# tari-project/bulletproofs-plus

Measured on AMD Instinct MI355X. Metric: 64-bit range proofs verified/sec (batch), higher is better.
Workload: dtype u32

## Files before the change

### bulletproofs-plus_amd/_build.py

```python
import os
import subprocess
import sys

HERE = os.path.dirname(os.path.abspath(__file__))
CSRC = os.path.join(HERE, "csrc")
LIB = os.path.join(HERE, "libbpp_hip.so")
HOSTTEST_LIB = os.path.join(HERE, "libbpp_hosttest.so")
SOURCES = ["engine.hip"]
HEADERS = sorted(f for f in os.listdir(CSRC) if f.endswith((".h", ".inc"))) + [os.path.join("..", "..", "include", "bpp.h")]


def _stale(target, deps):
    if not os.path.exists(target):
        return True
    t = os.path.getmtime(target)
    return any(os.path.getmtime(d) > t for d in deps if os.path.exists(d))


def hipcc_path():
    for cand in (os.environ.get("HIPCC"), "/opt/rocm/bin/hipcc", "hipcc"):
        if cand and (os.path.isabs(cand) and os.path.exists(cand) or not os.path.isabs(cand)):
            return cand
    return "hipcc"

# ... 189 lines not shown
def build_refill_mixed_harness(force=False):
    src = os.path.join(CSRC, "hosttest_refill_mixed.cpp")
    deps = [src] + [os.path.join(CSRC, h) for h in HEADERS]
    if not force and not _stale(REFILL_MIXED_SANITIZER_BIN, deps):
        return REFILL_MIXED_SANITIZER_BIN
    subprocess.run(["g++", "-O1", "-g", "-std=c++17", "-fsanitize=address,undefined", "-fno-sanitize-recover=undefined",
                    "-fno-omit-frame-pointer", "-o", REFILL_MIXED_SANITIZER_BIN, src], check=True, cwd=CSRC)
    return REFILL_MIXED_SANITIZER_BIN


ITEM_STATES_SANITIZER_BIN = os.path.join(HERE, "hosttest_item_states_asan")


def build_item_states_harness(force=False):
    src = os.path.join(CSRC, "hosttest_item_states.cpp")
    deps = [src] + [os.path.join(CSRC, h) for h in HEADERS]
    if not force and not _stale(ITEM_STATES_SANITIZER_BIN, deps):
        return ITEM_STATES_SANITIZER_BIN
    subprocess.run(["g++", "-O1", "-g", "-std=c++17", "-fsanitize=address,undefined", "-fno-sanitize-recover=undefined",
                    "-fno-omit-frame-pointer", "-o", ITEM_STATES_SANITIZER_BIN, src], check=True, cwd=CSRC)
    return ITEM_STATES_SANITIZER_BIN


if __name__ == "__main__":
    build(force="--force" in sys.argv, verbose=True)
    build_hosttest(force="--force" in sys.argv)
```

### bulletproofs-plus_amd/csrc/engine.hip

```cpp
#include <hip/hip_runtime.h>
#include <stdio.h>
#include <string.h>
#include <time.h>

#include <algorithm>
#include <array>
#include <atomic>
#include <chrono>
#include <condition_variable>
#include <deque>
#include <functional>
#include <map>
#include <set>
#include <memory>
#include <mutex>
#include <string>
#include <thread>
#include <vector>

#include "../../include/bpp.h"
#include "chain_dev.h"
#include "chain_host.h"
#include "ct.h"
#include "kernels_prove.h"
#include "kernels_verify.h"
#include "lanes_host.h"
#include "msm.h"
#include "msm_plain.h"
#include "prove_job_host.h"
#include "prove_pack_host.h"
#include "runtime_host.h"
#include "upload_host.h"
#include "ingest.h"
#include "ingest_mixed.h"
#include "verdict.h"
#include "refill.h"
#include "refill_mixed.h"
#include "item_states.h"

using namespace bpp;

namespace {

struct EngineError {
  int code;
  std::string msg;
};

#define HIP_CHECK(expr)                                                                          \
// ... 339 lines not shown
#define BPP_REFILLED_MSG "the batch was refilled on the stream (bpp_batch_refill_enqueue) and takes enqueued calls only: upload the arrays for a blocking call"

void adopt_buffers(Batch &dst, Batch &src) {
#define BPP_ADOPT(f) dst.f.swap(src.f)
  BPP_ADOPT(d_ext_status); BPP_ADOPT(bytes); BPP_ADOPT(states); BPP_ADOPT(seeds); BPP_ADOPT(d_desc); BPP_ADOPT(minvals);
  BPP_ADOPT(src_off); BPP_ADOPT(owner); BPP_ADOPT(idx_commit); BPP_ADOPT(idx_proof); BPP_ADOPT(status0); BPP_ADOPT(chal);
  BPP_ADOPT(rows); BPP_ADOPT(parts); BPP_ADOPT(gemm_lo); BPP_ADOPT(gemm_hi); BPP_ADOPT(gparts); BPP_ADOPT(gemm_mult); BPP_ADOPT(scal); BPP_ADOPT(shr); BPP_ADOPT(tab); BPP_ADOPT(rng_out); BPP_ADOPT(weights); BPP_ADOPT(chain_wide);
  BPP_ADOPT(masks); BPP_ADOPT(chal_bytes); BPP_ADOPT(status); BPP_ADOPT(group_first); BPP_ADOPT(group_dlo); BPP_ADOPT(dynpts); BPP_ADOPT(dyn_hi); BPP_ADOPT(dec_spill);
  BPP_ADOPT(msm.counts); BPP_ADOPT(msm.starts); BPP_ADOPT(msm.sorted); BPP_ADOPT(msm.order); BPP_ADOPT(msm.order_win);
  BPP_ADOPT(msm.cls_hist);
  BPP_ADOPT(msm.buckets); BPP_ADOPT(msm.Q); BPP_ADOPT(msm.W); BPP_ADOPT(msm.R); BPP_ADOPT(msm.comp32);
  BPP_ADOPT(msm.is_identity); BPP_ADOPT(msm.term_sidx); BPP_ADOPT(msm.term_pidx); BPP_ADOPT(msm.group_off);
  BPP_ADOPT(h_rng); BPP_ADOPT(h_weights); BPP_ADOPT(h_wide); BPP_ADOPT(h_status); BPP_ADOPT(h_status_any); BPP_ADOPT(h_ident); BPP_ADOPT(h_masks); BPP_ADOPT(h_states);
#undef BPP_ADOPT
  dst.h_status_dirty.swap(src.h_status_dirty);
  std::swap(dst.h_status_dirty_of, src.h_status_dirty_of);
  if (!src.status_settled) std::fill(dst.h_status_dirty.begin(), dst.h_status_dirty.end(), (uint8_t)1);
}

void wipe_batch_secrets(Batch &b, hipStream_t s);

}

struct PipeJob {
  uint64_t ticket = 0;
  int action = 0;
  size_t chunk = 0;
  std::shared_ptr<Params> Pp;
  uint64_t params = 0;
  UploadPlan pl;
  size_t n_items = 0;
  uint32_t t = 0;
  int rc = 0;
  std::string err;
  std::vector<uint8_t> masks, present;
  bool done = false;
};

struct PipeLane {
  bpp_ctx *child = nullptr;
  std::thread th;
  std::shared_ptr<PipeJob> job;
  bool busy = false;
};

struct Pipeline {
  std::mutex mu;
  std::condition_variable cv;
  std::mutex submit_mu;
  std::vector<std::unique_ptr<PipeLane>> lanes;
  std::map<uint64_t, std::shared_ptr<PipeJob>> tickets;
  uint64_t next_ticket = 1;
  uint32_t next_lane = 0;
  bool quit = false;
};

void pipeline_shutdown(bpp_ctx *ctx);

struct ProveJob;
using ProvePipeline = lanes::TicketLanes<bpp_ctx *, ProveJob>;
void prove_pipeline_shutdown(bpp_ctx *ctx);
int prove_pipeline_check_stats(bpp_ctx *ctx, struct bpp_prove_check_stats *sum);
int prove_pipeline_recovery_stats(bpp_ctx *ctx, uint64_t *replayed, uint64_t *mismatched);
int prove_pipeline_secret_bytes(bpp_ctx *ctx, uint64_t *examined, uint64_t *nonzero);

enum MsmReduce : uint32_t { MSM_RC_QUAD = 0, MSM_RC2 = 1, MSM_RC = 2, MSM_BITSUM = 3 };
struct MsmForm {
  bool valid = false;
  bool plain = false;
  bool ct = false;
  bool quad = false;
  MsmReduce reduce = MSM_RC_QUAD;
  bool final_quad = false;
  bool narrow = false;
  uint32_t dig_cap = 0;
  uint32_t slices = 0;
  uint32_t c = 0, K = 0, K_wide = 0, nb = 0, G = 0, terms = 0;
};

struct CtMsmWork {
// ... 42 lines not shown
  bool ev_wait_ready = false;
  WaitHint wait_hint_rng, wait_hint_end, wait_hint_prove;
  hipStream_t side_stream = nullptr;
  hipEvent_t ev_fork, ev_join;
  hipStream_t chain_stream = nullptr;
  hipEvent_t ev_chain_fork, ev_chain_done;
  DevBuf<Strobe> d_chain_t0;
  PinnedBuf<uint32_t> h_chain_zero;
  uint64_t device_chain_calls = 0, device_chain_redraws = 0, wide_chain_calls = 0;
  DevBuf<uint8_t> scratch128;
  DevBuf<uint8_t> prove_arena;
  PinnedBuf<uint8_t> prove_pin_in, prove_pin_out;
  std::vector<hipStream_t> prove_streams;
  std::vector<hipStream_t> prove_lane_streams;
  hipStream_t prove_msm_stream = nullptr;
  std::vector<hipEvent_t> prove_sync_events;
  std::vector<hipStream_t> prove_aux_streams;
  std::vector<hipEvent_t> prove_aux_events;
  std::vector<hipEvent_t> prove_events;
  bpp_prove_profile pprof{};
  struct Options {
    int transcripts_wave = -1, tables_wave = -1, side_decompress = -1, msm_c_bias = -1, msm_c_max = -1, msm_c_add = -1, msm_rc2 = -1, msm_quad = -1, msm_final_quad = -1,
        fb_threads = -1, prove_subs = -1, msm_split = -1, fused_columns = -1, prove_prio = -1, prove_fused = -1, static_gemm = -1, lazy_columns = -1, ct = -1, prove_parts = -1, prove_waves = -1, prove_fifo = -1, chain = -1, chain_test_zero = 0, wait = -1, ct_back = -1, chain_inline = -1, wide_in_lanes = -1,
        prove_check = -1, prove_check_recovery = -1, msm_plain = -1, verify_check = -1, msm_ct_k = -1, verify_joint = 0, msm_prelude_slices = 0;
  } opt;
  struct bpp_verify_check_stats vcheck_stats{};
  int verify_check_off = 0;
  struct bpp_verify_joint_stats vjoint_stats{};
  WaitHint wait_hint_fallback;
  struct VerifyTamper {
    int passes = 0, group = 0, kind = 0;
  } vtamper;
  std::unique_ptr<Batch> check_spare;
  WaitHint check_hint_rng, check_hint_end;
  struct bpp_prove_check_stats check_stats{};
  PinnedBuf<uint8_t> check_pin;
  DevBuf<uint8_t> check_dev;
  PinnedBuf<uint32_t> check_words;
  uint64_t check_replayed = 0, check_mismatched = 0;
  const void *check_zeroed_seeds = nullptr, *check_zeroed_masks = nullptr;
  size_t check_zeroed_seeds_n = 0, check_zeroed_masks_n = 0;
  std::mutex check_note_mu;
  std::vector<std::array<uint8_t, 32>> check_recovery_failed;
  struct CheckTamper {
    int proof = 0, byte = 1, mask = 1, times = 1, nonce = 0;
  } tamper;
  std::vector<hipEvent_t> enq_events;
// ... 38 lines not shown
    {"msm_split", "BPP_MSM_SPLIT", &bpp_ctx::Options::msm_split},
    {"fused_columns", "BPP_FUSED_COLUMNS", &bpp_ctx::Options::fused_columns},
    {"prove_prio", "BPP_PROVE_PRIO", &bpp_ctx::Options::prove_prio},
    {"prove_fused", "BPP_PROVE_FUSED", &bpp_ctx::Options::prove_fused},
    {"ct", "BPP_CT", &bpp_ctx::Options::ct},
    {"ct_back", "BPP_CT_BACK", &bpp_ctx::Options::ct_back},
    {"prove_parts", "BPP_PROVE_PARTS", &bpp_ctx::Options::prove_parts},
    {"prove_waves", "BPP_PROVE_WAVES", &bpp_ctx::Options::prove_waves},
    {"prove_fifo", "BPP_PROVE_FIFO", &bpp_ctx::Options::prove_fifo},
    {"static_gemm", "BPP_STATIC_GEMM", &bpp_ctx::Options::static_gemm},
    {"lazy_columns", "BPP_LAZY_COLUMNS", &bpp_ctx::Options::lazy_columns},
    {"chain", "BPP_CHAIN", &bpp_ctx::Options::chain},
    {"chain_test_zero", "BPP_CHAIN_TEST_ZERO", &bpp_ctx::Options::chain_test_zero},
    {"wait", "BPP_WAIT", &bpp_ctx::Options::wait},
    {"chain_inline", "BPP_CHAIN_INLINE", &bpp_ctx::Options::chain_inline},
    {"wide_in_lanes", "BPP_WIDE_IN_LANES", &bpp_ctx::Options::wide_in_lanes},
    {"prove_check", "BPP_PROVE_CHECK", &bpp_ctx::Options::prove_check},
    {"prove_check_recovery", "BPP_PROVE_CHECK_RECOVERY", &bpp_ctx::Options::prove_check_recovery},
    {"msm_plain", "BPP_MSM_PLAIN", &bpp_ctx::Options::msm_plain},
    {"verify_check", "BPP_VERIFY_CHECK", &bpp_ctx::Options::verify_check},
    {"msm_ct_k", "BPP_MSM_CT_K", &bpp_ctx::Options::msm_ct_k},
    {"verify_joint", "BPP_VERIFY_JOINT", &bpp_ctx::Options::verify_joint},
    {"msm_prelude_slices", "BPP_MSM_PRELUDE_SLICES", &bpp_ctx::Options::msm_prelude_slices},
};
struct TamperName {
  const char *name;
  int bpp_ctx::CheckTamper::*field;
};
const TamperName kTamperKnobs[] = {
    {"prove_check_tamper", &bpp_ctx::CheckTamper::proof},
    {"prove_check_tamper_byte", &bpp_ctx::CheckTamper::byte},
    {"prove_check_tamper_xor", &bpp_ctx::CheckTamper::mask},
    {"prove_check_tamper_times", &bpp_ctx::CheckTamper::times},
    {"prove_check_tamper_nonce", &bpp_ctx::CheckTamper::nonce},
};
struct VerifyTamperName {
  const char *name;
  int bpp_ctx::VerifyTamper::*field;
};
const VerifyTamperName kVerifyTamperKnobs[] = {
    {"verify_check_tamper", &bpp_ctx::VerifyTamper::passes},
    {"verify_check_tamper_group", &bpp_ctx::VerifyTamper::group},
    {"verify_check_tamper_kind", &bpp_ctx::VerifyTamper::kind},
};
void options_from_env(bpp_ctx *c) {
  for (const OptionName &o : kOptions)
// ... 981 lines not shown
  std::vector<uint32_t> first(n_groups + 1);
  for (size_t g = 0; g <= n_groups; g++) first[g] = (uint32_t)(g * n_per_group);
  run_weight_chains_generic(rng32_all, weights32_out, first.data(), (uint32_t)n_groups);
  return BPP_OK;
}

int bpp_weights_from_chain(const uint8_t *rng32_all, size_t n_total, uint8_t *weights32_out) {
  if ((!rng32_all || !weights32_out) && n_total) return BPP_ERR_INVALID_ARGUMENT;
  weights_from_chain_host(rng32_all, n_total, weights32_out);
  return BPP_OK;
}

}

namespace {

void wipe_batch_secrets(Batch &b, hipStream_t s) {
  if (b.seeds.p && b.seeds_dirty) (void)hipMemsetAsync(b.seeds.p, 0, b.seeds.n, s);
  if (b.masks.p && b.masks_dirty) (void)hipMemsetAsync(b.masks.p, 0, b.masks.n, s);
  b.seeds_dirty = b.masks_dirty = false;
}

void upload_host_pack(bpp_ctx *ctx, const Params &P, const bpp_verify_item *items, size_t n_items, const bpp_packed_batch *packed,
                      UploadPlan &pl) {
  const ParallelFor pf = [](uint32_t n, const std::function<void(uint32_t)> &fn) { host_parallel_for(n, fn); };
  const ParamShape shape{P.n_bits, P.m_max, P.t};
  std::vector<bpp_verify_item> synth;
  const bool arithmetic = packed && upload_pass_a_packed(*packed, pl, pf);
  if (packed && !arithmetic) {
    upload_packed_as_items(*packed, synth);
    items = synth.data();
    n_items = synth.size();
  }
  if (!arithmetic) upload_pass_a(items, n_items, pl);
  ctx->pin_upload.resize(pl.bytes_total + BPP_BYTES_SLACK);
  uint8_t *bytes = ctx->pin_upload.data();
  memset(bytes + pl.bytes_total, 0, BPP_BYTES_SLACK);
  if (arithmetic) upload_pass_b_packed(*packed, shape, pl, bytes, pf);
  else upload_pass_b(items, shape, pl, bytes, pf);
}

std::unique_ptr<Batch> new_batch(bpp_ctx *ctx) {
  auto B = std::make_unique<Batch>();
  if (ctx->spare_batch) {
    adopt_buffers(*B, *ctx->spare_batch);
    ctx->spare_batch.reset();
  }
  return B;
}

uint64_t upload_device(bpp_ctx *ctx, const std::shared_ptr<Params> &Pp, uint64_t params, UploadPlan &pl,
                       const uint8_t *const *challenges32, const uint8_t *rng_out32, std::unique_ptr<Batch> filled = nullptr) {
    Params &P = *Pp;
    const size_t n_items = pl.n_items;
    const bool resident = filled != nullptr;
    std::unique_ptr<Batch> B = resident ? std::move(filled) : new_batch(ctx);
    hipStream_t s = ctx->stream;
    SmallStaging L;
    bool registered = false;
// ... 2013 lines not shown
  *out = ctx->enq_stats;
  return BPP_OK;
}

int bpp_verify_batch_with_challenges(bpp_ctx *ctx, uint64_t params, const bpp_verify_item *items, size_t n_items,
                                     const uint8_t *const *challenges32, const uint8_t *rng_out32, int action, size_t chunk,
                                     uint8_t *masks_out, uint8_t *mask_present, char *errbuf, size_t errbuf_len) {
  auto upload = [&](uint64_t *h) -> int {
    BPP_ENTRY(ctx);
    if (!challenges32 || !rng_out32) return fail(ctx, BPP_ERR_INVALID_ARGUMENT, "null argument", errbuf, errbuf_len);
    return upload_impl(ctx, params, items, n_items, nullptr, h, challenges32, rng_out32, errbuf, errbuf_len);
  };
  return verify_uploaded(ctx, n_items, upload, action, chunk, masks_out, mask_present, errbuf, errbuf_len);
}

int bpp_verify_batch(bpp_ctx *ctx, uint64_t params, const bpp_verify_item *items, size_t n_items, int action,
                     size_t chunk, uint8_t *masks_out, uint8_t *mask_present, char *errbuf, size_t errbuf_len) {
  auto upload = [&](uint64_t *h) -> int { return bpp_batch_upload(ctx, params, items, n_items, h, errbuf, errbuf_len); };
  return verify_uploaded(ctx, n_items, upload, action, chunk, masks_out, mask_present, errbuf, errbuf_len);
}

int bpp_verify_batch_packed(bpp_ctx *ctx, uint64_t params, const bpp_packed_batch *in, int action, size_t chunk,
                            uint8_t *masks_out, uint8_t *mask_present, char *errbuf, size_t errbuf_len) {
  auto upload = [&](uint64_t *h) -> int { return bpp_batch_upload_packed(ctx, params, in, h, errbuf, errbuf_len); };
  return verify_uploaded(ctx, in ? in->n_items : SIZE_MAX, upload, action, chunk, masks_out, mask_present, errbuf, errbuf_len);
}

int bpp_verify_batch_packed_device(bpp_ctx *ctx, uint64_t params, const bpp_packed_batch *in, int action, size_t chunk,
                                   uint8_t *masks_out, uint8_t *mask_present, char *errbuf, size_t errbuf_len) {
  auto upload = [&](uint64_t *h) -> int { return bpp_batch_upload_packed_device(ctx, params, in, h, errbuf, errbuf_len); };
  return verify_uploaded(ctx, in ? in->n_items : SIZE_MAX, upload, action, chunk, masks_out, mask_present, errbuf, errbuf_len);
}

int bpp_verify_batch_mixed(bpp_ctx *ctx, uint64_t params, const bpp_mixed_batch *in, int action, size_t chunk, uint8_t *masks_out,
                           uint8_t *mask_present, char *errbuf, size_t errbuf_len) {
  auto upload = [&](uint64_t *h) -> int { return bpp_batch_upload_mixed(ctx, params, in, h, errbuf, errbuf_len); };
  return verify_uploaded(ctx, in ? in->n_items : SIZE_MAX, upload, action, chunk, masks_out, mask_present, errbuf, errbuf_len);
}

int bpp_verify_batch_mixed_device(bpp_ctx *ctx, uint64_t params, const bpp_mixed_batch *in, int action, size_t chunk,
                                  uint8_t *masks_out, uint8_t *mask_present, char *errbuf, size_t errbuf_len) {
  auto upload = [&](uint64_t *h) -> int { return bpp_batch_upload_mixed_device(ctx, params, in, h, errbuf, errbuf_len); };
  return verify_uploaded(ctx, in ? in->n_items : SIZE_MAX, upload, action, chunk, masks_out, mask_present, errbuf, errbuf_len);
}

int bpp_verify_batch_states(bpp_ctx *ctx, uint64_t params, const bpp_verify_item *items, size_t n_items, int action, size_t chunk,
// ... 85 lines not shown
  std::lock_guard<std::mutex> lk(init_mu);
  return slot;
}

template <class P, class F>
void pipeline_end(std::mutex &init_mu, std::shared_ptr<P> &slot, F on_uncollected) {
  std::shared_ptr<P> pp;
  {
    std::lock_guard<std::mutex> lk(init_mu);
    pp = std::move(slot);
    slot.reset();
  }
  if (!pp) return;
  pp->shutdown(on_uncollected);
  pp->for_each_lane([](bpp_ctx *c) { bpp_ctx_destroy(c); });
}

void pipe_worker(bpp_ctx *owner, Pipeline *pp, PipeLane *lane) {
  (void)hipSetDevice(owner->device);
  for (;;) {
    std::shared_ptr<PipeJob> job;
    {
      std::unique_lock<std::mutex> lk(pp->mu);
      pp->cv.wait(lk, [&] { return pp->quit || lane->job; });
      if (!lane->job) return;
      job = std::move(lane->job);
      lane->job.reset();
    }
    bpp_ctx *c = lane->child;
    char err[256];
    err[0] = 0;
    uint64_t h = 0;
    int rc = BPP_OK;
    GateHold gate(device_state(owner->device), job->n_items <= BPP_GATE_SMALL_PROOFS);
    {
      std::lock_guard<std::mutex> lk(c->mu);
      try {
        h = upload_device(c, job->Pp, job->params, job->pl, nullptr, nullptr);
      } catch (const EngineError &e) {
        rc = fail(c, e.code, e.msg, err, sizeof(err));
      } catch (const ProofErr &e) {
        rc = fail(c, e.code, e.msg, err, sizeof(err));
      } catch (const std::exception &e) {
        rc = fail(c, BPP_ERR_ENGINE, e.what(), err, sizeof(err));
      }
    }
    if (rc == BPP_OK) {
      const bool want_masks = job->action != BPP_VERIFY_ONLY;
      if (want_masks) {
        job->masks.assign(job->n_items * job->t * 32, 0);
        job->present.assign(job->n_items, 0);
      }
      rc = bpp_verify_resident(c, h, job->action, job->chunk, want_masks ? job->masks.data() : nullptr,
                               want_masks ? job->present.data() : nullptr, err, sizeof(err));
      (void)bpp_batch_destroy(c, h);
    }
    {
      std::lock_guard<std::mutex> lk(pp->mu);
      job->rc = rc;
      job->err = err;
      job->done = true;
      lane->busy = false;
    }
    pp->cv.notify_all();
  }
}

std::shared_ptr<Pipeline> make_pipeline(bpp_ctx *owner, const std::vector<bpp_ctx *> &children) {
  auto pp = std::make_shared<Pipeline>();
  for (bpp_ctx *c : children) {
    pp->lanes.push_back(std::make_unique<PipeLane>());
    pp->lanes.back()->child = c;
  }
  try {
    for (auto &lane : pp->lanes) lane->th = std::thread(pipe_worker, owner, pp.get(), lane.get());
  } catch (...) {
    {
      std::lock_guard<std::mutex> lk(pp->mu);
      pp->quit = true;
    }
    pp->cv.notify_all();
    for (auto &lane : pp->lanes)
      if (lane->th.joinable()) lane->th.join();
    throw;
  }
// ... 4 lines not shown

void pipeline_shutdown(bpp_ctx *ctx) {
  std::shared_ptr<Pipeline> pp;
  {
    std::lock_guard<std::mutex> lk(ctx->pipe_init_mu);
    pp = std::move(ctx->pipe);
    ctx->pipe.reset();
  }
  if (!pp) return;
  {
    std::unique_lock<std::mutex> lk(pp->mu);
    pp->cv.wait(lk, [&] {
      for (auto &l : pp->lanes)
        if (l->busy) return false;
      return true;
    });
    pp->quit = true;
  }
  pp->cv.notify_all();
  for (auto &l : pp->lanes) {
    if (l->th.joinable()) l->th.join();
    bpp_ctx_destroy(l->child);
  }
  std::lock_guard<std::mutex> lk(pp->mu);
  for (auto &kv : pp->tickets) wipe(kv.second->masks.data(), kv.second->masks.size());
  pp->tickets.clear();
}

extern "C" {

int bpp_ctx_pipeline_depth(bpp_ctx *ctx, uint32_t depth) {
  if (!ctx) return BPP_ERR_BAD_HANDLE;
  std::lock_guard<std::mutex> lk(ctx->pipe_init_mu);
  if (ctx->pipe) return fail(ctx, BPP_ERR_INVALID_ARGUMENT, "the pipeline is already running");
  if (depth < 1 || depth > 16) return fail(ctx, BPP_ERR_INVALID_ARGUMENT, "pipeline depth must be 1..16");
  ctx->pipe_depth = depth;
  return BPP_OK;
}

int bpp_verify_submit_packed(bpp_ctx *ctx, uint64_t params, const bpp_packed_batch *in, int action, size_t chunk,
                             uint64_t *ticket, char *errbuf, size_t errbuf_len) {
  if (!ctx) return BPP_ERR_BAD_HANDLE;
  if (hipSetDevice(ctx->device) != hipSuccess) return BPP_ERR_NO_DEVICE;
  try {
    if (!in || !ticket || in->n_items == 0)
      return fail(nullptr, BPP_ERR_INVALID_ARGUMENT, "Range statements or proofs length empty", errbuf, errbuf_len);
    if (action < 0 || action > 2) return fail(nullptr, BPP_ERR_INVALID_ARGUMENT, "unknown verify action", errbuf, errbuf_len);
    if (in->n_items > (1u << 24)) return fail(nullptr, BPP_ERR_SIZE_OVERFLOW, "batch too large", errbuf, errbuf_len);
    const std::shared_ptr<Params> Pp = params_registry().get(params);
    if (!Pp || Pp->device != ctx->device) return fail(nullptr, BPP_ERR_BAD_HANDLE, "unknown params handle", errbuf, errbuf_len);
    const std::shared_ptr<Pipeline> pp = pipeline_get(ctx, ctx->pipe_init_mu, ctx->pipe, ctx->pipe_depth, "pipeline lane: context creation failed",
                                                      [&](const std::vector<bpp_ctx *> &children) { return make_pipeline(ctx, children); });
    std::lock_guard<std::mutex> submit_lock(pp->submit_mu);
    PipeLane *lane;
    {
      std::unique_lock<std::mutex> lk(pp->mu);
      lane = pp->lanes[pp->next_lane].get();
      pp->cv.wait(lk, [&] { return !lane->busy; });
      lane->busy = true;
      pp->next_lane = (pp->next_lane + 1) % (uint32_t)pp->lanes.size();
    }
    auto job = std::make_shared<PipeJob>();
    job->action = action;
    job->chunk = chunk;
    job->Pp = Pp;
    job->params = params;
    job->n_items = in->n_items;
    job->t = Pp->t;
    try {
      upload_host_pack(lane->child, *Pp, nullptr, 0, in, job->pl);
    } catch (...) {
      secure_wipe(job->pl.seeds.data(), job->pl.seeds.size());
      {
        std::lock_guard<std::mutex> lk(pp->mu);
        lane->busy = false;
      }
      pp->cv.notify_all();
      throw;
    }
    {
      std::lock_guard<std::mutex> lk(pp->mu);
      job->ticket = pp->next_ticket++;
      pp->tickets[job->ticket] = job;
      lane->job = job;
      *ticket = job->ticket;
    }
    pp->cv.notify_all();
    return BPP_OK;
  }
  BPP_CATCH(nullptr, errbuf, errbuf_len)
}

int bpp_verify_collect(bpp_ctx *ctx, uint64_t ticket, uint8_t *masks_out, uint8_t *mask_present, char *errbuf,
                       size_t errbuf_len) {
  if (!ctx) return BPP_ERR_BAD_HANDLE;
  const std::shared_ptr<Pipeline> pp = pipeline_peek(ctx->pipe_init_mu, ctx->pipe);
  if (!pp) return fail(nullptr, BPP_ERR_BAD_HANDLE, "unknown ticket", errbuf, errbuf_len);
  std::shared_ptr<PipeJob> job;
  {
    std::unique_lock<std::mutex> lk(pp->mu);
    auto it = pp->tickets.find(ticket);
    if (it == pp->tickets.end()) return fail(nullptr, BPP_ERR_BAD_HANDLE, "unknown ticket", errbuf, errbuf_len);
    job = it->second;
    pp->cv.wait(lk, [&] { return job->done; });
    if (!pp->tickets.erase(ticket)) return fail(nullptr, BPP_ERR_BAD_HANDLE, "unknown ticket", errbuf, errbuf_len);
  }
  ScopeExit wipe_masks{[&] { wipe(job->masks.data(), job->masks.size()); }};
  if (job->rc != BPP_OK) {
    set_err(errbuf, errbuf_len, job->err);
    return job->rc;
  }
  const size_t n = job->n_items, t = job->t;
  const bool have = job->action != BPP_VERIFY_ONLY;
  if (mask_present) {
    if (have) memcpy(mask_present, job->present.data(), n);
    else memset(mask_present, 0, n);
  }
  if (masks_out) {
    if (have) memcpy(masks_out, job->masks.data(), n * t * 32);
    else memset(masks_out, 0, n * t * 32);
  }
  return BPP_OK;
}

int bpp_verify_phase1(bpp_ctx *ctx, uint64_t batch, uint8_t *rng_out32, char *errbuf, size_t errbuf_len) {
  BPP_ENTRY(ctx);
  try {
    auto it = ctx->batches.find(batch);
    if (it == ctx->batches.end()) return fail(ctx, BPP_ERR_BAD_HANDLE, "unknown batch handle", errbuf, errbuf_len);
    Batch &b = *it->second;
    if (b.refilled) return fail(ctx, BPP_ERR_INVALID_ARGUMENT, BPP_REFILLED_MSG, errbuf, errbuf_len);
    StageTimer tm(ctx);
    layout_groups(ctx, b, 0);
    if (b.any_defer) check_deferred(b.defer, 0, b.B);
    enqueue_phase1(ctx, b, tm, b.any_rounds_bad);
    fetch_status(ctx, b);
    HIP_CHECK(hipStreamSynchronize(ctx->stream));
    if (rng_out32) memcpy(rng_out32, b.h_rng.data(), (size_t)b.B * 32);
    check_chunk_errors(b, 0, b.B);
    b.phase1_done = true;
    return BPP_OK;
  }
  BPP_CATCH(ctx, errbuf, errbuf_len)
}

// ... 314 lines not shown
```

Measured before the change: 27.81 million.

## Split large packed verify batches into parts overlapped across helper lanes

Large blocking packed-verify calls are cut into up to four chunk-aligned parts. Each part is host-packed into double-buffered pinned staging and queued on its own worker lane with a separate context, so host packing of one part overlaps device verification of earlier ones. Per-part results and stats are then folded back together. This adds helper threads and contexts, extra pinned memory and more complex error/secret-wipe handling, and splitting may shrink per-launch batch size.

```diff
diff --git a/bulletproofs-plus_amd/_build.py b/bulletproofs-plus_amd/_build.py
--- a/bulletproofs-plus_amd/_build.py
+++ b/bulletproofs-plus_amd/_build.py
@@ -235,6 +235,18 @@
     return ITEM_STATES_SANITIZER_BIN
 
 
+OVERLAP_SANITIZER_BIN = os.path.join(HERE, "hosttest_overlap_asan")
+
+
+def build_overlap_harness(force=False):
+    src = os.path.join(CSRC, "hosttest_overlap.cpp")
+    if not force and not _stale(OVERLAP_SANITIZER_BIN, [src, os.path.join(CSRC, "overlap_host.h")]):
+        return OVERLAP_SANITIZER_BIN
+    subprocess.run(["g++", "-O1", "-g", "-std=c++17", "-pthread", "-fsanitize=address,undefined", "-fno-sanitize-recover=undefined",
+                    "-fno-omit-frame-pointer", "-o", OVERLAP_SANITIZER_BIN, src], check=True, cwd=CSRC)
+    return OVERLAP_SANITIZER_BIN
+
+
 if __name__ == "__main__":
     build(force="--force" in sys.argv, verbose=True)
     build_hosttest(force="--force" in sys.argv)
diff --git a/bulletproofs-plus_amd/csrc/engine.hip b/bulletproofs-plus_amd/csrc/engine.hip
--- a/bulletproofs-plus_amd/csrc/engine.hip
+++ b/bulletproofs-plus_amd/csrc/engine.hip
@@ -25,6 +25,7 @@
 #include "kernels_prove.h"
 #include "kernels_verify.h"
 #include "lanes_host.h"
+#include "overlap_host.h"
 #include "msm.h"
 #include "msm_plain.h"
 #include "prove_job_host.h"
@@ -410,6 +411,7 @@
 
 }
 
+struct PipeLane;
 struct PipeJob {
   uint64_t ticket = 0;
   int action = 0;
@@ -423,13 +425,32 @@
   std::string err;
   std::vector<uint8_t> masks, present;
   bool done = false;
+  PipeLane *home = nullptr;
+  std::vector<std::shared_ptr<PipeJob>> parts;
+  std::vector<overlap::Part> cuts;
+  uint32_t parts_left = 0;
+  PipeJob *whole = nullptr;
+  PinnedBuf<uint8_t> *staging = nullptr;
+  bool is_part = false;
+  struct bpp_verify_check_stats d_vcheck{};
+  struct bpp_verify_joint_stats d_vjoint{};
+  std::vector<uint8_t> &seeds() { return pl.seeds; }
+  bool finished() const {
+    if (parts.empty()) return done;
+    for (auto &p : parts)
+      if (!p->done) return false;
+    return true;
+  }
 };
 
 struct PipeLane {
   bpp_ctx *child = nullptr;
   std::thread th;
-  std::shared_ptr<PipeJob> job;
+  std::deque<std::shared_ptr<PipeJob>> queue;
   bool busy = false;
+  PinnedBuf<uint8_t> part_staging[2];
+  std::shared_ptr<PipeJob> staging_user[2];
+  uint32_t next_slot = 0;
 };
 
 struct Pipeline {
@@ -437,6 +458,7 @@
   std::condition_variable cv;
   std::mutex submit_mu;
   std::vector<std::unique_ptr<PipeLane>> lanes;
+  std::vector<std::unique_ptr<PipeLane>> helpers;
   std::map<uint64_t, std::shared_ptr<PipeJob>> tickets;
   uint64_t next_ticket = 1;
   uint32_t next_lane = 0;
@@ -444,6 +466,12 @@
 };
 
 void pipeline_shutdown(bpp_ctx *ctx);
+#define BPP_OVERLAP_MAX_WORKERS 4u
+namespace {
+uint32_t overlap_parts_of_call(bpp_ctx *ctx, uint64_t params, const bpp_packed_batch *in, int action, size_t chunk, bool blocking);
+}
+int verify_packed_overlapped(bpp_ctx *ctx, uint64_t params, const bpp_packed_batch *in, int action, size_t chunk, uint32_t n_parts,
+                             uint8_t *masks_out, uint8_t *mask_present, char *errbuf, size_t errbuf_len);
 
 struct ProveJob;
 using ProvePipeline = lanes::TicketLanes<bpp_ctx *, ProveJob>;
@@ -532,7 +560,7 @@
   struct Options {
     int transcripts_wave = -1, tables_wave = -1, side_decompress = -1, msm_c_bias = -1, msm_c_max = -1, msm_c_add = -1, msm_rc2 = -1, msm_quad = -1, msm_final_quad = -1,
         fb_threads = -1, prove_subs = -1, msm_split = -1, fused_columns = -1, prove_prio = -1, prove_fused = -1, static_gemm = -1, lazy_columns = -1, ct = -1, prove_parts = -1, prove_waves = -1, prove_fifo = -1, chain = -1, chain_test_zero = 0, wait = -1, ct_back = -1, chain_inline = -1, wide_in_lanes = -1,
-        prove_check = -1, prove_check_recovery = -1, msm_plain = -1, verify_check = -1, msm_ct_k = -1, verify_joint = 0, msm_prelude_slices = 0;
+        prove_check = -1, prove_check_recovery = -1, msm_plain = -1, verify_check = -1, msm_ct_k = -1, verify_joint = 0, msm_prelude_slices = 0, verify_overlap = -1;
   } opt;
   struct bpp_verify_check_stats vcheck_stats{};
   int verify_check_off = 0;
@@ -617,6 +645,7 @@
     {"msm_ct_k", "BPP_MSM_CT_K", &bpp_ctx::Options::msm_ct_k},
     {"verify_joint", "BPP_VERIFY_JOINT", &bpp_ctx::Options::verify_joint},
     {"msm_prelude_slices", "BPP_MSM_PRELUDE_SLICES", &bpp_ctx::Options::msm_prelude_slices},
+    {"verify_overlap", "BPP_VERIFY_OVERLAP", &bpp_ctx::Options::verify_overlap},
 };
 struct TamperName {
   const char *name;
@@ -1644,7 +1673,7 @@
 }
 
 void upload_host_pack(bpp_ctx *ctx, const Params &P, const bpp_verify_item *items, size_t n_items, const bpp_packed_batch *packed,
-                      UploadPlan &pl) {
+                      UploadPlan &pl, PinnedBuf<uint8_t> *staging = nullptr) {
   const ParallelFor pf = [](uint32_t n, const std::function<void(uint32_t)> &fn) { host_parallel_for(n, fn); };
   const ParamShape shape{P.n_bits, P.m_max, P.t};
   std::vector<bpp_verify_item> synth;
@@ -1655,8 +1684,9 @@
     n_items = synth.size();
   }
   if (!arithmetic) upload_pass_a(items, n_items, pl);
-  ctx->pin_upload.resize(pl.bytes_total + BPP_BYTES_SLACK);
-  uint8_t *bytes = ctx->pin_upload.data();
+  PinnedBuf<uint8_t> &pin = staging ? *staging : ctx->pin_upload;
+  pin.resize(pl.bytes_total + BPP_BYTES_SLACK);
+  uint8_t *bytes = pin.data();
   memset(bytes + pl.bytes_total, 0, BPP_BYTES_SLACK);
   if (arithmetic) upload_pass_b_packed(*packed, shape, pl, bytes, pf);
   else upload_pass_b(items, shape, pl, bytes, pf);
@@ -3716,6 +3746,9 @@
 
 int bpp_verify_batch_packed(bpp_ctx *ctx, uint64_t params, const bpp_packed_batch *in, int action, size_t chunk,
                             uint8_t *masks_out, uint8_t *mask_present, char *errbuf, size_t errbuf_len) {
+  if (!ctx) return BPP_ERR_BAD_HANDLE;
+  const uint32_t n_parts = overlap_parts_of_call(ctx, params, in, action, chunk, true);
+  if (n_parts >= 2) return verify_packed_overlapped(ctx, params, in, action, chunk, n_parts, masks_out, mask_present, errbuf, errbuf_len);
   auto upload = [&](uint64_t *h) -> int { return bpp_batch_upload_packed(ctx, params, in, h, errbuf, errbuf_len); };
   return verify_uploaded(ctx, in ? in->n_items : SIZE_MAX, upload, action, chunk, masks_out, mask_present, errbuf, errbuf_len);
 }
@@ -3847,10 +3880,10 @@
     std::shared_ptr<PipeJob> job;
     {
       std::unique_lock<std::mutex> lk(pp->mu);
-      pp->cv.wait(lk, [&] { return pp->quit || lane->job; });
-      if (!lane->job) return;
-      job = std::move(lane->job);
-      lane->job.reset();
+      pp->cv.wait(lk, [&] { return pp->quit || !lane->queue.empty(); });
+      if (lane->queue.empty()) return;
+      job = std::move(lane->queue.front());
+      lane->queue.pop_front();
     }
     bpp_ctx *c = lane->child;
     char err[256];
@@ -3858,8 +3891,18 @@
     uint64_t h = 0;
     int rc = BPP_OK;
     GateHold gate(device_state(owner->device), job->n_items <= BPP_GATE_SMALL_PROOFS);
+    struct bpp_verify_check_stats vcheck0{};
+    struct bpp_verify_joint_stats vjoint0{};
     {
       std::lock_guard<std::mutex> lk(c->mu);
+      if (job->is_part) {
+        vcheck0 = c->vcheck_stats;
+        vjoint0 = c->vjoint_stats;
+      }
+      if (job->staging) c->pin_upload.swap(*job->staging);
+      ScopeExit staging_back{[&] {
+        if (job->staging) c->pin_upload.swap(*job->staging);
+      }};
       try {
         h = upload_device(c, job->Pp, job->params, job->pl, nullptr, nullptr);
       } catch (const EngineError &e) {
@@ -3880,12 +3923,29 @@
                                want_masks ? job->present.data() : nullptr, err, sizeof(err));
       (void)bpp_batch_destroy(c, h);
     }
+    if (job->is_part) {
+      std::lock_guard<std::mutex> lk(c->mu);
+      auto take = [](uint64_t &now, uint64_t before, uint64_t &delta) {
+        delta = now - before;
+        now = before;
+      };
+      take(c->vcheck_stats.calls, vcheck0.calls, job->d_vcheck.calls);
+      take(c->vcheck_stats.rechecked_groups, vcheck0.rechecked_groups, job->d_vcheck.rechecked_groups);
+      take(c->vcheck_stats.confirmed, vcheck0.confirmed, job->d_vcheck.confirmed);
+      take(c->vcheck_stats.overturned, vcheck0.overturned, job->d_vcheck.overturned);
+      take(c->vcheck_stats.tie_breaks, vcheck0.tie_breaks, job->d_vcheck.tie_breaks);
+      take(c->vcheck_stats.undecided, vcheck0.undecided, job->d_vcheck.undecided);
+      take(c->vjoint_stats.calls, vjoint0.calls, job->d_vjoint.calls);
+      take(c->vjoint_stats.accepted, vjoint0.accepted, job->d_vjoint.accepted);
+      take(c->vjoint_stats.fallbacks, vjoint0.fallbacks, job->d_vjoint.fallbacks);
+      take(c->vjoint_stats.fallback_all_ok, vjoint0.fallback_all_ok, job->d_vjoint.fallback_all_ok);
+    }
     {
       std::lock_guard<std::mutex> lk(pp->mu);
       job->rc = rc;
       job->err = err;
       job->done = true;
-      lane->busy = false;
+      if (!job->whole || --job->whole->parts_left == 0) job->home->busy = false;
     }
     pp->cv.notify_all();
   }
@@ -3936,24 +3996,56 @@
     if (l->th.joinable()) l->th.join();
     bpp_ctx_destroy(l->child);
   }
+  for (auto &h : pp->helpers) {
+    if (h->th.joinable()) h->th.join();
+    bpp_ctx_destroy(h->child);
+  }
   std::lock_guard<std::mutex> lk(pp->mu);
-  for (auto &kv : pp->tickets) wipe(kv.second->masks.data(), kv.second->masks.size());
+  for (auto &kv : pp->tickets) {
+    wipe(kv.second->masks.data(), kv.second->masks.size());
+    for (auto &part : kv.second->parts) wipe(part->masks.data(), part->masks.size());
+  }
   pp->tickets.clear();
 }
 
-extern "C" {
-
-int bpp_ctx_pipeline_depth(bpp_ctx *ctx, uint32_t depth) {
-  if (!ctx) return BPP_ERR_BAD_HANDLE;
-  std::lock_guard<std::mutex> lk(ctx->pipe_init_mu);
-  if (ctx->pipe) return fail(ctx, BPP_ERR_INVALID_ARGUMENT, "the pipeline is already running");
-  if (depth < 1 || depth > 16) return fail(ctx, BPP_ERR_INVALID_ARGUMENT, "pipeline depth must be 1..16");
-  ctx->pipe_depth = depth;
-  return BPP_OK;
-}
-
-int bpp_verify_submit_packed(bpp_ctx *ctx, uint64_t params, const bpp_packed_batch *in, int action, size_t chunk,
-                             uint64_t *ticket, char *errbuf, size_t errbuf_len) {
+namespace {
+
+uint32_t overlap_parts_of_call(bpp_ctx *ctx, uint64_t params, const bpp_packed_batch *in, int action, size_t chunk, bool blocking) {
+  if (!in || in->n_items < 2 || in->n_items > (1u << 24) || action < 0 || action > 2 || chunk == 0) return 1;
+  const uint64_t n = in->n_items;
+  if (n * in->proof_len + n * in->m * 32 >= (1ull << 32) || n * in->m >= (1ull << 28) || n * ((uint64_t)in->m + 3 + 2 * BPP_MAX_WIRE_ROUNDS) >= (1ull << 31))
+    return 1;
+  const std::shared_ptr<Params> Pp = params_registry().get(params);
+  if (!Pp || Pp->device != ctx->device) return 1;
+  int option, joint;
+  uint32_t depth;
+  {
+    std::lock_guard<std::mutex> lk(ctx->mu);
+    if (ctx->vtamper.passes) return 1;
+    option = ctx->opt.verify_overlap;
+    joint = ctx->opt.verify_joint;
+  }
+  {
+    std::lock_guard<std::mutex> lk(ctx->pipe_init_mu);
+    depth = ctx->pipe_depth;
+  }
+  return overlap::parts_for(option, in->n_items, chunk, blocking || depth == 1, joint > 0);
+}
+
+bpp_packed_batch packed_item_range(const bpp_packed_batch &in, const overlap::Part &p) {
+  bpp_packed_batch sub = in;
+  sub.n_items = p.n_items;
+  if (in.proofs) sub.proofs = in.proofs + p.item0 * in.proof_stride;
+  if (in.commitments32) sub.commitments32 = in.commitments32 + p.item0 * (size_t)in.m * 32;
+  if (in.min_values) sub.min_values = in.min_values + p.item0 * (size_t)in.m;
+  if (in.min_present) sub.min_present = in.min_present + p.item0 * (size_t)in.m;
+  if (in.seed_nonces32) sub.seed_nonces32 = in.seed_nonces32 + p.item0 * 32;
+  if (in.seed_present) sub.seed_present = in.seed_present + p.item0;
+  return sub;
+}
+
+int verify_submit_packed(bpp_ctx *ctx, uint64_t params, const bpp_packed_batch *in, int action, size_t chunk, uint32_t n_parts,
+                         uint64_t *ticket, char *errbuf, size_t errbuf_len) {
   if (!ctx) return BPP_ERR_BAD_HANDLE;
   if (hipSetDevice(ctx->device) != hipSuccess) return BPP_ERR_NO_DEVICE;
   try {
@@ -3965,6 +4057,8 @@
     if (!Pp || Pp->device != ctx->device) return fail(nullptr, BPP_ERR_BAD_HANDLE, "unknown params handle", errbuf, errbuf_len);
     const std::shared_ptr<Pipeline> pp = pipeline_get(ctx, ctx->pipe_init_mu, ctx->pipe, ctx->pipe_depth, "pipeline lane: context creation failed",
                                                       [&](const std::vector<bpp_ctx *> &children) { return make_pipeline(ctx, children); });
+    bpp_ctx::Options opt_now;
+    if (n_parts >= 2) opt_now = ctx_options(ctx);
     std::lock_guard<std::mutex> submit_lock(pp->submit_mu);
     PipeLane *lane;
     {
@@ -3974,29 +4068,112 @@
       lane->busy = true;
       pp->next_lane = (pp->next_lane + 1) % (uint32_t)pp->lanes.size();
     }
-    auto job = std::make_shared<PipeJob>();
-    job->action = action;
-    job->chunk = chunk;
-    job->Pp = Pp;
-    job->params = params;
-    job->n_items = in->n_items;
-    job->t = Pp->t;
-    try {
-      upload_host_pack(lane->child, *Pp, nullptr, 0, in, job->pl);
-    } catch (...) {
-      secure_wipe(job->pl.seeds.data(), job->pl.seeds.size());
+    auto release = [&] {
       {
         std::lock_guard<std::mutex> lk(pp->mu);
         lane->busy = false;
       }
       pp->cv.notify_all();
-      throw;
+    };
+    auto new_job = [&](size_t n_items) {
+      auto job = std::make_shared<PipeJob>();
+      job->action = action;
+      job->chunk = chunk;
+      job->Pp = Pp;
+      job->params = params;
+      job->n_items = n_items;
+      job->t = Pp->t;
+      return job;
+    };
+    auto job = new_job(in->n_items);
+    job->home = lane;
+    if (n_parts >= 2) {
+      job->cuts = overlap::split(in->n_items, chunk, n_parts);
+      for (const overlap::Part &p : job->cuts) {
+        job->parts.push_back(new_job(p.n_items));
+        job->parts.back()->is_part = true;
+        job->parts.back()->whole = job.get();
+        job->parts.back()->home = lane;
+      }
+      job->parts_left = (uint32_t)job->parts.size();
+      const uint32_t W = std::min<uint32_t>((uint32_t)job->parts.size(), BPP_OVERLAP_MAX_WORKERS);
+      try {
+        while (pp->helpers.size() + 1 < W) {
+          std::vector<bpp_ctx *> made;
+          if (make_lane_contexts(ctx->device, 1, nullptr, [&](bpp_ctx *c) { c->opt = opt_now; }, made) != BPP_OK)
+            throw EngineError{BPP_ERR_ENGINE, "pipeline lane: context creation failed"};
+          auto helper = std::make_unique<PipeLane>();
+          helper->child = made[0];
+          try {
+            helper->th = std::thread(pipe_worker, ctx, pp.get(), helper.get());
+          } catch (...) {
+            bpp_ctx_destroy(made[0]);
+            throw;
+          }
+          pp->helpers.push_back(std::move(helper));
+        }
+      } catch (...) {
+        release();
+        throw;
+      }
+      auto worker_of = [&](size_t k) { return k % W ? pp->helpers[k % W - 1].get() : lane; };
+      for (uint32_t w = 0; w < W; w++) {
+        bpp_ctx *c = worker_of(w)->child;
+        std::lock_guard<std::mutex> lk(c->mu);
+        c->opt = opt_now;
+      }
+      auto drain = [&](size_t n) {
+        std::unique_lock<std::mutex> lk(pp->mu);
+        pp->cv.wait(lk, [&] {
+          for (size_t k = 0; k < n; k++)
+            if (!job->parts[k]->done) return false;
+          return true;
+        });
+      };
+      try {
+        overlap::submit_parts(
+            job->parts,
+            [&](size_t k, PipeJob &part) {
+              PipeLane *w = worker_of(k);
+              const uint32_t slot = w->next_slot;
+              if (std::shared_ptr<PipeJob> &user = w->staging_user[slot]) {
+                std::unique_lock<std::mutex> lk(pp->mu);
+                pp->cv.wait(lk, [&] { return user->done; });
+                user.reset();
+              }
+              part.staging = &w->part_staging[slot];
+              const bpp_packed_batch sub = packed_item_range(*in, job->cuts[k]);
+              upload_host_pack(w->child, *Pp, nullptr, 0, &sub, part.pl, part.staging);
+            },
+            [&](size_t k, PipeJob &) {
+              PipeLane *w = worker_of(k);
+              w->staging_user[w->next_slot] = job->parts[k];
+              w->next_slot ^= 1u;
+              {
+                std::lock_guard<std::mutex> lk(pp->mu);
+                w->queue.push_back(job->parts[k]);
+              }
+              pp->cv.notify_all();
+            },
+            drain);
+      } catch (...) {
+        release();
+        throw;
+      }
+    } else {
+      try {
+        upload_host_pack(lane->child, *Pp, nullptr, 0, in, job->pl);
+      } catch (...) {
+        secure_wipe(job->pl.seeds.data(), job->pl.seeds.size());
+        release();
+        throw;
+      }
     }
     {
       std::lock_guard<std::mutex> lk(pp->mu);
       job->ticket = pp->next_ticket++;
       pp->tickets[job->ticket] = job;
-      lane->job = job;
+      if (job->parts.empty()) lane->queue.push_back(job);
       *ticket = job->ticket;
     }
     pp->cv.notify_all();
@@ -4005,8 +4182,7 @@
   BPP_CATCH(nullptr, errbuf, errbuf_len)
 }
 
-int bpp_verify_collect(bpp_ctx *ctx, uint64_t ticket, uint8_t *masks_out, uint8_t *mask_present, char *errbuf,
-                       size_t errbuf_len) {
+int verify_collect(bpp_ctx *ctx, uint64_t ticket, uint8_t *masks_out, uint8_t *mask_present, char *errbuf, size_t errbuf_len) {
   if (!ctx) return BPP_ERR_BAD_HANDLE;
   const std::shared_ptr<Pipeline> pp = pipeline_peek(ctx->pipe_init_mu, ctx->pipe);
   if (!pp) return fail(nullptr, BPP_ERR_BAD_HANDLE, "unknown ticket", errbuf, errbuf_len);
@@ -4016,8 +4192,25 @@
     auto it = pp->tickets.find(ticket);
     if (it == pp->tickets.end()) return fail(nullptr, BPP_ERR_BAD_HANDLE, "unknown ticket", errbuf, errbuf_len);
     job = it->second;
-    pp->cv.wait(lk, [&] { return job->done; });
+    pp->cv.wait(lk, [&] { return job->finished(); });
     if (!pp->tickets.erase(ticket)) return fail(nullptr, BPP_ERR_BAD_HANDLE, "unknown ticket", errbuf, errbuf_len);
+  }
+  const bool have = job->action != BPP_VERIFY_ONLY;
+  if (!job->parts.empty()) {
+    {
+      std::lock_guard<std::mutex> lk(ctx->mu);
+      struct bpp_verify_check_stats v{};
+      for (auto &p : job->parts) {
+        add_stats(v, p->d_vcheck);
+        add_stats(ctx->vjoint_stats, p->d_vjoint);
+      }
+      v.calls = v.calls ? 1 : 0;
+      add_stats(ctx->vcheck_stats, v);
+    }
+    std::string err;
+    const int rc = overlap::fold_parts(job->parts, job->cuts, (size_t)job->t * 32, have, masks_out, mask_present, BPP_OK, err);
+    if (rc != BPP_OK) set_err(errbuf, errbuf_len, err);
+    return rc;
   }
   ScopeExit wipe_masks{[&] { wipe(job->masks.data(), job->masks.size()); }};
   if (job->rc != BPP_OK) {
@@ -4025,7 +4218,6 @@
     return job->rc;
   }
   const size_t n = job->n_items, t = job->t;
-  const bool have = job->action != BPP_VERIFY_ONLY;
   if (mask_present) {
     if (have) memcpy(mask_present, job->present.data(), n);
     else memset(mask_present, 0, n);
@@ -4035,6 +4227,45 @@
     else memset(masks_out, 0, n * t * 32);
   }
   return BPP_OK;
+}
+
+}
+
+int verify_packed_overlapped(bpp_ctx *ctx, uint64_t params, const bpp_packed_batch *in, int action, size_t chunk, uint32_t n_parts,
+                             uint8_t *masks_out, uint8_t *mask_present, char *errbuf, size_t errbuf_len) {
+  char err[256];
+  err[0] = 0;
+  uint64_t ticket = 0;
+  int rc = verify_submit_packed(ctx, params, in, action, chunk, n_parts, &ticket, err, sizeof(err));
+  if (rc == BPP_OK) rc = verify_collect(ctx, ticket, masks_out, mask_present, err, sizeof(err));
+  if (rc != BPP_OK) {
+    std::lock_guard<std::mutex> lk(ctx->mu);
+    return fail(ctx, rc, err, errbuf, errbuf_len);
+  }
+  return BPP_OK;
+}
+
+extern "C" {
+
+int bpp_ctx_pipeline_depth(bpp_ctx *ctx, uint32_t depth) {
+  if (!ctx) return BPP_ERR_BAD_HANDLE;
+  std::lock_guard<std::mutex> lk(ctx->pipe_init_mu);
+  if (ctx->pipe) return fail(ctx, BPP_ERR_INVALID_ARGUMENT, "the pipeline is already running");
+  if (depth < 1 || depth > 16) return fail(ctx, BPP_ERR_INVALID_ARGUMENT, "pipeline depth must be 1..16");
+  ctx->pipe_depth = depth;
+  return BPP_OK;
+}
+
+int bpp_verify_submit_packed(bpp_ctx *ctx, uint64_t params, const bpp_packed_batch *in, int action, size_t chunk,
+                             uint64_t *ticket, char *errbuf, size_t errbuf_len) {
+  if (!ctx) return BPP_ERR_BAD_HANDLE;
+  const uint32_t n_parts = ticket ? overlap_parts_of_call(ctx, params, in, action, chunk, false) : 1;
+  return verify_submit_packed(ctx, params, in, action, chunk, n_parts, ticket, errbuf, errbuf_len);
+}
+
+int bpp_verify_collect(bpp_ctx *ctx, uint64_t ticket, uint8_t *masks_out, uint8_t *mask_present, char *errbuf,
+                       size_t errbuf_len) {
+  return verify_collect(ctx, ticket, masks_out, mask_present, errbuf, errbuf_len);
 }
 
 int bpp_verify_phase1(bpp_ctx *ctx, uint64_t batch, uint8_t *rng_out32, char *errbuf, size_t errbuf_len) {
diff --git a/bulletproofs-plus_amd/csrc/hosttest_overlap.cpp b/bulletproofs-plus_amd/csrc/hosttest_overlap.cpp
--- /dev/null
+++ b/bulletproofs-plus_amd/csrc/hosttest_overlap.cpp
@@ -0,0 +1,309 @@
+#include "overlap_host.h"
+
+#include <condition_variable>
+#include <cstdio>
+#include <cstdlib>
+#include <deque>
+#include <mutex>
+#include <stdexcept>
+#include <thread>
+
+namespace {
+
+int g_failed = 0;
+#define CHECK(cond)                                                      \
+  do {                                                                   \
+    if (!(cond)) {                                                       \
+      printf("FAILED %s:%d: %s\n", __FILE__, __LINE__, #cond);           \
+      g_failed++;                                                        \
+    }                                                                    \
+  } while (0)
+
+const int OK = 0, REJECTED = 1, CONSTRUCTION = 2;
+const size_t ROW = 32;
+
+struct Job {
+  int rc = OK;
+  std::string err;
+  std::vector<uint8_t> masks, present, nonce_bytes, staged;
+  std::vector<uint8_t> &seeds() { return nonce_bytes; }
+  overlap::Part part;
+  bool done = false, ran = false;
+};
+
+bool all_zero(const std::vector<uint8_t> &v) {
+  for (uint8_t b : v)
+    if (b) return false;
+  return true;
+}
+
+struct FakeLane {
+  std::mutex mu;
+  std::condition_variable cv;
+  std::deque<std::shared_ptr<Job>> queue;
+  bool quit = false;
+  size_t chunk;
+  bool want_masks;
+  std::vector<size_t> order;
+  std::thread th;
+
+  FakeLane(size_t chunk_, bool want_masks_) : chunk(chunk_), want_masks(want_masks_) { th = std::thread([this] { work(); }); }
+  ~FakeLane() {
+    {
+      std::lock_guard<std::mutex> lk(mu);
+      quit = true;
+    }
+    cv.notify_all();
+    th.join();
+  }
+  void post(std::shared_ptr<Job> j) {
+    {
+      std::lock_guard<std::mutex> lk(mu);
+      queue.push_back(std::move(j));
+    }
+    cv.notify_all();
+  }
+  void drain(const std::vector<std::shared_ptr<Job>> &jobs, size_t n) {
+    std::unique_lock<std::mutex> lk(mu);
+    cv.wait(lk, [&] {
+      for (size_t k = 0; k < n; k++)
+        if (!jobs[k]->done) return false;
+      return true;
+    });
+  }
+  void work() {
+    for (;;) {
+      std::shared_ptr<Job> j;
+      {
+        std::unique_lock<std::mutex> lk(mu);
+        cv.wait(lk, [&] { return quit || !queue.empty(); });
+        if (queue.empty()) return;
+        j = queue.front();
+        queue.pop_front();
+      }
+      const size_t n = j->part.n_items;
+      std::vector<uint8_t> had_nonce(n, 0);
+      for (size_t i = 0; i < n; i++) had_nonce[i] = !j->nonce_bytes.empty() && j->nonce_bytes[i * 32] == 0xA5;
+      overlap::wipe_bytes(j->nonce_bytes);
+      int rc = OK;
+      std::string err;
+      for (size_t i = 0; i < n && rc == OK; i++)
+        if (j->staged[i] == 1) {
+          rc = REJECTED;
+          err = "rejected group " + std::to_string((j->part.item0 + i) / chunk);
+        }
+      if (rc == OK && want_masks) {
+        j->masks.assign(n * ROW, 0);
+        j->present.assign(n, 0);
+        for (size_t i = 0; i < n; i++)
+          if (had_nonce[i]) {
+            j->present[i] = 1;
+            memset(&j->masks[i * ROW], (int)((j->part.item0 + i) & 0xff) | 0x80, ROW);
+          }
+      } else if (want_masks) {
+        j->masks.assign(n * ROW, 0x77);
+        j->present.assign(n, 0);
+      }
+      {
+        std::lock_guard<std::mutex> lk(mu);
+        j->rc = rc;
+        j->err = err;
+        j->ran = j->done = true;
+        order.push_back(j->part.item0);
+      }
+      cv.notify_all();
+    }
+  }
+};
+
+struct ConstructionError {
+  size_t index;
+};
+
+struct Outcome {
+  int rc = OK;
+  std::string err;
+  std::vector<uint8_t> masks, present;
+  bool operator==(const Outcome &o) const { return rc == o.rc && err == o.err && masks == o.masks && present == o.present; }
+};
+
+Outcome reference(const std::vector<uint8_t> &items, const std::vector<uint8_t> &nonce, size_t chunk, bool want_masks) {
+  Outcome o;
+  o.masks.assign(items.size() * ROW, 0xEE);
+  o.present.assign(items.size(), 0xEE);
+  for (size_t i = 0; i < items.size(); i++)
+    if (items[i] == 2) {
+      o.rc = CONSTRUCTION;
+      o.err = "construction error at item " + std::to_string(i);
+      return o;
+    }
+  for (size_t i = 0; i < items.size(); i++)
+    if (items[i] == 1) {
+      o.rc = REJECTED;
+      o.err = "rejected group " + std::to_string(i / chunk);
+      return o;
+    }
+  for (size_t i = 0; i < items.size(); i++) {
+    const bool p = want_masks && nonce[i];
+    o.present[i] = p;
+    memset(&o.masks[i * ROW], p ? (int)(i & 0xff) | 0x80 : 0, ROW);
+  }
+  return o;
+}
+
+struct RunInfo {
+  std::vector<std::shared_ptr<Job>> jobs;
+  std::vector<size_t> order;
+  size_t drained = (size_t)-1;
+};
+
+Outcome run_split(const std::vector<uint8_t> &items, const std::vector<uint8_t> &nonce, size_t chunk, uint32_t P, bool want_masks, RunInfo &info) {
+  Outcome o;
+  o.masks.assign(items.size() * ROW, 0xEE);
+  o.present.assign(items.size(), 0xEE);
+  const std::vector<overlap::Part> cuts = overlap::split(items.size(), chunk, P);
+  std::vector<std::shared_ptr<Job>> jobs;
+  for (const overlap::Part &p : cuts) {
+    jobs.push_back(std::make_shared<Job>());
+    jobs.back()->part = p;
+  }
+  {
+    FakeLane lane(chunk, want_masks);
+    try {
+      overlap::submit_parts(
+          jobs,
+          [&](size_t k, Job &j) {
+            const overlap::Part &p = cuts[k];
+            j.nonce_bytes.assign(p.n_items * 32, 0);
+            for (size_t i = 0; i < p.n_items; i++) {
+              if (nonce[p.item0 + i]) memset(&j.nonce_bytes[i * 32], 0xA5, 32);
+              if (items[p.item0 + i] == 2) throw ConstructionError{p.item0 + i};
+              j.staged.push_back(items[p.item0 + i]);
+            }
+          },
+          [&](size_t k, Job &) { lane.post(jobs[k]); },
+          [&](size_t n) {
+            info.drained = n;
+            lane.drain(jobs, n);
+            for (size_t k = 0; k < n; k++) CHECK(jobs[k]->ran);
+          });
+      lane.drain(jobs, jobs.size());
+      o.rc = overlap::fold_parts(jobs, cuts, ROW, want_masks, o.masks.data(), o.present.data(), OK, o.err);
+    } catch (const ConstructionError &e) {
+      o.rc = CONSTRUCTION;
+      o.err = "construction error at item " + std::to_string(e.index);
+    }
+    info.order = lane.order;
+  }
+  info.jobs = jobs;
+  return o;
+}
+
+void no_secret_left(const RunInfo &info) {
+  for (auto &j : info.jobs) {
+    CHECK(all_zero(j->nonce_bytes));
+    CHECK(all_zero(j->masks));
+  }
+}
+
+void test_split() {
+  for (size_t chunk : {1, 4, 1024})
+    for (size_t G = 1; G <= 70; G++)
+      for (size_t tail : {(size_t)0, (size_t)1, chunk - 1})
+        for (uint32_t P : {1u, 2u, 3u, 4u, 8u, 64u, 200u}) {
+          if (tail >= chunk) continue;
+          const size_t n = G * chunk - tail;
+          if (overlap::groups_of(n, chunk) != G) continue;
+          const std::vector<overlap::Part> parts = overlap::split(n, chunk, P);
+          CHECK(parts.size() == std::min<size_t>(P, G));
+          size_t item = 0, group = 0;
+          for (size_t k = 0; k < parts.size(); k++) {
+            const overlap::Part &p = parts[k];
+            CHECK(p.item0 == item && p.group0 == group && p.n_groups >= 1 && p.n_items >= 1);
+            CHECK(p.item0 % chunk == 0);
+            CHECK(k == 0 || p.n_groups <= parts[k - 1].n_groups);
+            CHECK(parts[0].n_groups - p.n_groups <= 1);
+            CHECK(overlap::groups_of(p.n_items, chunk) == p.n_groups);
+            item += p.n_items;
+            group += p.n_groups;
+          }
+          CHECK(item == n && group == G);
+        }
+  printf("ok split\n");
+}
+
+void test_rule() {
+  using overlap::parts_for;
+  const size_t big = 64 * 1024;
+  CHECK(parts_for(0, big, 1024, true, false) == 1 && parts_for(1, big, 1024, true, false) == 1);
+  CHECK(parts_for(4, big, 0, true, false) == 1 && parts_for(4, big, (size_t)-1, true, false) == 1);
+  CHECK(parts_for(4, big, 1024, true, true) == 1 && parts_for(-1, big, 1024, true, true) == 1);
+  CHECK(parts_for(4, 32, 4, false, false) == 4 && parts_for(3, 28, 4, false, false) == 3);
+  CHECK(parts_for(8, 12, 4, false, false) == 3 && parts_for(4, 4, 4, false, false) == 1);
+  CHECK(parts_for(1000, big * 4, 1024, false, false) == overlap::MAX_PARTS);
+  CHECK(parts_for(-1, big, 1024, false, false) == 1);
+  CHECK(parts_for(-1, 32, 4, true, false) == 1 && parts_for(-1, 1024, 1024, true, false) == 1);
+  const uint32_t by_rule = parts_for(-1, big, 1024, true, false);
+  CHECK(by_rule == (overlap::RULE_PARTS >= 2 ? overlap::RULE_PARTS : 1u));
+  if (overlap::RULE_PARTS >= 2) {
+    CHECK(parts_for(-1, overlap::RULE_MIN_GROUPS * (size_t)1024, 1024, true, false) == overlap::RULE_PARTS || overlap::RULE_MIN_GROUPS * (size_t)1024 < overlap::RULE_MIN_PROOFS);
+    CHECK(parts_for(-1, (overlap::RULE_MIN_GROUPS - 1) * (size_t)1024, 1024, true, false) == 1);
+  }
+  printf("ok rule\n");
+}
+
+void compare(const char *name, const std::vector<uint8_t> &items, const std::vector<uint8_t> &nonce, size_t chunk, uint32_t P, bool want_masks,
+             size_t want_drained) {
+  RunInfo info;
+  const Outcome got = run_split(items, nonce, chunk, P, want_masks, info);
+  const Outcome want = reference(items, nonce, chunk, want_masks);
+  CHECK(got == want);
+  CHECK(info.drained == want_drained);
+  for (size_t k = 1; k < info.order.size(); k++) CHECK(info.order[k - 1] < info.order[k]);
+  no_secret_left(info);
+  printf("ok %s\n", name);
+}
+
+}
+
+int main() {
+  test_split();
+  test_rule();
+  const size_t NONE = (size_t)-1;
+  std::vector<uint8_t> valid(32, 0), nonce(32, 0), no_nonce(32, 0);
+  for (size_t i = 0; i < 32; i += 3) nonce[i] = 1;
+  compare("fold_all_valid", valid, no_nonce, 4, 4, false, NONE);
+  compare("fold_masks", valid, nonce, 4, 4, true, NONE);
+  compare("fold_masks_7_groups_4_parts", std::vector<uint8_t>(28, 0), std::vector<uint8_t>(28, 1), 4, 4, true, NONE);
+  compare("fold_short_last_group", std::vector<uint8_t>(30, 0), std::vector<uint8_t>(30, 1), 4, 3, true, NONE);
+  {
+    std::vector<uint8_t> v = valid;
+    v[5 * 4 + 1] = 1;
+    compare("fold_one_rejected", v, nonce, 4, 4, true, NONE);
+    v[1 * 4 + 2] = 1;
+    v[6 * 4] = 1;
+    compare("fold_lowest_group_wins", v, nonce, 4, 4, true, NONE);
+    compare("fold_lowest_group_wins_verify_only", v, nonce, 4, 8, false, NONE);
+  }
+  {
+    std::vector<uint8_t> v = valid;
+    v[1] = 1;
+    v[6 * 4 + 3] = 2;
+    compare("drain_construction_error_part_3", v, nonce, 4, 4, true, 3);
+    v[2 * 4] = 2;
+    compare("drain_lowest_construction_error", v, nonce, 4, 4, true, 1);
+    v[0] = 2;
+    compare("drain_nothing_posted", v, nonce, 4, 4, true, 0);
+  }
+  {
+    std::vector<uint8_t> v = valid;
+    v[31] = 2;
+    compare("drain_last_item", v, std::vector<uint8_t>(32, 1), 4, 2, true, 1);
+  }
+  if (g_failed) {
+    printf("%d check(s) failed\n", g_failed);
+    return 1;
+  }
+  printf("all ok\n");
+  return 0;
+}
diff --git a/bulletproofs-plus_amd/csrc/overlap_host.h b/bulletproofs-plus_amd/csrc/overlap_host.h
--- /dev/null
+++ b/bulletproofs-plus_amd/csrc/overlap_host.h
@@ -0,0 +1,106 @@
+#pragma once
+#include <stddef.h>
+#include <stdint.h>
+#include <string.h>
+
+#include <algorithm>
+#include <memory>
+#include <string>
+#include <vector>
+
+namespace overlap {
+
+constexpr uint32_t RULE_PARTS = 4;
+constexpr uint32_t RULE_MIN_GROUPS = 32;
+constexpr size_t RULE_MIN_PROOFS = 32768;
+constexpr uint32_t MAX_PARTS = 64;
+
+struct Part {
+  size_t item0 = 0, n_items = 0;
+  uint32_t group0 = 0, n_groups = 0;
+};
+
+inline size_t groups_of(size_t n_items, size_t chunk) {
+  if (chunk == 0 || chunk == (size_t)-1 || n_items == 0) return n_items ? 1 : 0;
+  return (n_items + chunk - 1) / chunk;
+}
+
+inline uint32_t parts_for(int option, size_t n_items, size_t chunk, bool unhidden, bool joint) {
+  if (chunk == 0 || chunk == (size_t)-1 || joint || option == 0 || option == 1) return 1;
+  const size_t G = groups_of(n_items, chunk);
+  if (G < 2) return 1;
+  if (option >= 2) return (uint32_t)std::min<size_t>({(size_t)option, G, (size_t)MAX_PARTS});
+  if (!unhidden || G < RULE_MIN_GROUPS || n_items < RULE_MIN_PROOFS || RULE_PARTS < 2) return 1;
+  return (uint32_t)std::min<size_t>(RULE_PARTS, G);
+}
+
+inline std::vector<Part> split(size_t n_items, size_t chunk, uint32_t P) {
+  std::vector<Part> parts;
+  const size_t G = groups_of(n_items, chunk);
+  if (P < 1) P = 1;
+  if ((size_t)P > G) P = (uint32_t)G;
+  uint32_t g = 0;
+  for (uint32_t k = 0; k < P; k++) {
+    Part p;
+    p.group0 = g;
+    p.n_groups = (uint32_t)(G / P + (k < G % P ? 1 : 0));
+    p.item0 = (size_t)g * chunk;
+    g += p.n_groups;
+    p.n_items = std::min(n_items, (size_t)g * chunk) - p.item0;
+    parts.push_back(p);
+  }
+  return parts;
+}
+
+inline void wipe_bytes(std::vector<uint8_t> &v) {
+  if (!v.empty()) explicit_bzero(v.data(), v.size());
+}
+
+template <class Job, class Pack, class Post, class Drain>
+void submit_parts(std::vector<std::shared_ptr<Job>> &jobs, Pack pack, Post post, Drain drain) {
+  size_t posted = 0;
+  try {
+    for (size_t k = 0; k < jobs.size(); k++) {
+      pack(k, *jobs[k]);
+      post(k, *jobs[k]);
+      posted = k + 1;
+    }
+  } catch (...) {
+    for (size_t k = posted; k < jobs.size(); k++) wipe_bytes(jobs[k]->seeds());
+    drain(posted);
+    for (size_t k = 0; k < posted; k++) wipe_bytes(jobs[k]->masks);
+    throw;
+  }
+}
+
+template <class Job>
+int fold_parts(const std::vector<std::shared_ptr<Job>> &jobs, const std::vector<Part> &parts, size_t mask_row_bytes, bool have_masks,
+               uint8_t *masks_out, uint8_t *mask_present, int ok_code, std::string &err) {
+  struct WipeAll {
+    const std::vector<std::shared_ptr<Job>> &jobs;
+    ~WipeAll() {
+      for (auto &j : jobs) wipe_bytes(j->masks);
+    }
+  } wipe_all{jobs};
+  for (size_t k = 0; k < jobs.size(); k++)
+    if (jobs[k]->rc != ok_code) {
+      err = jobs[k]->err;
+      return jobs[k]->rc;
+    }
+  for (size_t k = 0; k < jobs.size(); k++) {
+    const Part &p = parts[k];
+    const Job &j = *jobs[k];
+    const bool have = have_masks && j.masks.size() >= p.n_items * mask_row_bytes && j.present.size() >= p.n_items;
+    if (mask_present) {
+      if (have) memcpy(mask_present + p.item0, j.present.data(), p.n_items);
+      else memset(mask_present + p.item0, 0, p.n_items);
+    }
+    if (masks_out) {
+      if (have) memcpy(masks_out + p.item0 * mask_row_bytes, j.masks.data(), p.n_items * mask_row_bytes);
+      else memset(masks_out + p.item0 * mask_row_bytes, 0, p.n_items * mask_row_bytes);
+    }
+  }
+  return ok_code;
+}
+
+}
```

New measurement: 27.69 million. No clear change (-0.4%).
